# loicland/superpoint_graph

Hardware: NVIDIA H100
Metric: spg_train_step_edges_plus_points_per_sec (higher is better)
Workload: dtype f32

## Files before the change

### superpoint_graph_b200/csrc/tc_gemm2.cu

```cuda
#include <cuda.h>
#include <stdlib.h>

#include <mutex>

#include "common.cuh"
#include "tc_common.cuh"

namespace spg {

constexpr int T2_BM = 128;
constexpr int T2_KC = 32;
constexpr int T2_MAX_STAGES = 4;
constexpr int T2_EPI_WARPS = 8, T2_PROD_WARPS = 8;
constexpr int T2_THREADS = (T2_EPI_WARPS + T2_PROD_WARPS) * 32;
constexpr int T2_A_BYTES = T2_BM * T2_KC * 4;
constexpr int T2_STAGE_BYTES = 2 * T2_A_BYTES;

enum { PRO_AFFINE = 0, PRO_BNBWD = 1 };
enum { EPI_NONE = 0, EPI_STATS = 1, EPI_BNRED = 2 };

struct Tc2Args {
    const float* A;
    int64_t lda;
    const float* A2;
    int64_t lda2;
    const float* bias;
    float* C;
    int64_t ldc;
    int64_t M;
    int N, K;
    const float *a_scale, *a_shift;
    int a_relu;
    const float *a_mean, *a_var, *a_s12;
    float a_eps;
    float* dy_out;
    int64_t lddy;
    int epi;
    float* part;
    float *mean_out, *var_out;
    FoldArgs fold;
    const float* e_y;
    int64_t e_ldy;
    const float *e_scale, *e_shift, *e_mean, *e_var;
    float e_eps;
    int e_relu;
    float* e_s12;
    int nstages;
};

__device__ __forceinline__ void tma_load_2d(uint32_t dst, const CUtensorMap* map, int x, int y, uint32_t bar) {
    asm volatile(
        "cp.async.bulk.tensor.2d.shared::cluster.global.mbarrier::complete_tx::bytes [%0], [%1, {%2, %3}], [%4];"
        ::"r"(dst), "l"(map), "r"(x), "r"(y), "r"(bar)
        : "memory");
}

template <int NS, int PRO>
__global__ void __launch_bounds__(T2_THREADS, 1)
tc_gemm2_kernel(const Tc2Args p, const __grid_constant__ CUtensorMap wmap) {
    extern __shared__ __align__(1024) uint8_t smem_raw[];
    uint8_t* smem = smem_raw;
    if ((smem_u32(smem_raw) & 1023u) != 0u) __trap();
    __shared__ __align__(8) uint64_t bars[2 * T2_MAX_STAGES + 1];

    const int t = threadIdx.x;
    const int warp = t >> 5, lane = t & 31;
    const int nk = p.K / T2_KC;
    const int n0 = blockIdx.y * NS;
    const int64_t tiles = (p.M + T2_BM - 1) / T2_BM;
    const int nst = p.nstages;
    uint8_t* wres = smem + (size_t)nst * T2_STAGE_BYTES;

    const uint32_t bars_u32 = smem_u32(&bars[0]);
    auto bar_full = [&](int s) { return bars_u32 + 8u * (uint32_t)s; };
    auto bar_empty = [&](int s) { return bars_u32 + 8u * (uint32_t)(T2_MAX_STAGES + s); };
    const uint32_t bar_w = bars_u32 + 8u * (2 * T2_MAX_STAGES);

    if (t == 0) {
#pragma unroll
        for (int s = 0; s < T2_MAX_STAGES; ++s) {
            mbar_init(bar_full(s), T2_PROD_WARPS);
            mbar_init(bar_empty(s), T2_EPI_WARPS);
        }
        mbar_init(bar_w, 1);
        asm volatile("fence.mbarrier_init.release.cluster;" ::: "memory");
        asm volatile("prefetch.tensormap [%0];" ::"l"(&wmap) : "memory");
    }
    SPG_PDL_ENTRY();
    if (t == 0) {
        mbar_expect_tx(bar_w, (uint32_t)(nk * 2 * NS * T2_KC * 4));
        const uint32_t wres_u = smem_u32(wres);
        for (int blk = 0; blk < nk * 2; ++blk)
            tma_load_2d(wres_u + (uint32_t)blk * (NS * T2_KC * 4), &wmap, 0, blk * p.N + n0, bar_w);
    }
    constexpr int PF = PRO == PRO_BNBWD ? 2 : 4;
    constexpr int NOPS = PRO == PRO_BNBWD ? 2 : 1;
    float4 q[PF][NOPS][4];
    const int pt = t - T2_EPI_WARPS * 32;
    auto load = [&](int64_t tile, int kc, float4 (&dst)[NOPS][4]) {
        const int64_t m0 = tile * T2_BM;
#pragma unroll
        for (int j = 0; j < 4; ++j) {
            const int i = pt + 256 * j;
            const int row = i >> 3, c16 = i & 7;
            const bool ok = tile < tiles && m0 + row < p.M;
            dst[0][j] = ok ? __ldg(reinterpret_cast<const float4*>(p.A + (m0 + row) * p.lda + kc * T2_KC + c16 * 4))
                           : make_float4(0.f, 0.f, 0.f, 0.f);
            if (PRO == PRO_BNBWD)
                dst[NOPS - 1][j] =
                    ok ? __ldg(reinterpret_cast<const float4*>(p.A2 + (m0 + row) * p.lda2 + kc * T2_KC + c16 * 4))
                       : make_float4(0.f, 0.f, 0.f, 0.f);
        }
    };
    auto advance = [&](int64_t& tl, int& k) {
        if (++k == nk) {
            k = 0;
            tl += gridDim.x;
        }
    };
    int64_t ltile = blockIdx.x;
    int lkc = 0;
    if (pt >= 0) {
#pragma unroll
        for (int d = 0; d < PF - 1; ++d) {
            load(ltile, lkc, q[d]);
            advance(ltile, lkc);
        }
    }
    float* sc_s = reinterpret_cast<float*>(wres + (size_t)nk * 2 * NS * T2_KC * 4);
    float* sh_s = sc_s + p.K;
    float* cy_s = sh_s + p.K;
    float* c0_s = cy_s + p.K;
    float* bias_s = c0_s + p.K;
    float* ev_s = bias_s + NS;
    float* acc_s = ev_s + 4 * NS;
    for (int i = t; i < p.K; i += T2_THREADS) {
        const float sc = p.a_scale ? p.a_scale[i] : 1.f;
        sc_s[i] = sc;
        sh_s[i] = p.a_shift ? p.a_shift[i] : 0.f;
        if (PRO == PRO_BNBWD) {
            const float mu = p.a_mean[i], rstd = 1.f / sqrtf(p.a_var[i] + p.a_eps);
            const float m1 = p.a_s12[i] / (float)p.M, m2 = p.a_s12[p.K + i] / (float)p.M;
            cy_s[i] = -sc * rstd * m2;
            c0_s[i] = sc * (rstd * m2 * mu - m1);
        }
    }
    for (int i = t; i < NS; i += T2_THREADS) {
        bias_s[i] = p.bias ? p.bias[n0 + i] : 0.f;
        if (p.epi == EPI_BNRED) {
            ev_s[i] = p.e_scale ? p.e_scale[n0 + i] : 1.f;
            ev_s[NS + i] = p.e_shift ? p.e_shift[n0 + i] : 0.f;
            ev_s[2 * NS + i] = p.e_mean[n0 + i];
            ev_s[3 * NS + i] = 1.f / sqrtf(p.e_var[n0 + i] + p.e_eps);
        }
    }
    for (int i = t; i < T2_EPI_WARPS * NS * 4; i += T2_THREADS) acc_s[i] = 0.f;
    __syncthreads();

    if (warp >= T2_EPI_WARPS) {
        const bool pro = PRO == PRO_BNBWD || p.a_scale || p.a_shift || p.a_relu;
        int64_t tile = blockIdx.x;
        int kc = 0;
        uint32_t it = 0;
        const int c16 = pt & 7;
        uint32_t soff[4];
#pragma unroll
        for (int j = 0; j < 4; ++j) soff[j] = sw128_off((pt >> 3) + 32 * j, c16);
        const uint32_t smem_u = smem_u32(smem);
        const bool side_store = PRO == PRO_BNBWD && p.dy_out != nullptr && blockIdx.y == 0;
        auto st_shared4 = [](uint32_t addr, uint4 v) {
            asm volatile("st.shared.v4.b32 [%0], {%1, %2, %3, %4};" ::"r"(addr), "r"(v.x), "r"(v.y),
                         "r"(v.z), "r"(v.w)
                         : "memory");
        };
        auto consume = [&](float4 (&cur)[NOPS][4], float4 (&far)[NOPS][4]) {
            const int s = it % nst;
            const uint32_t use = it / nst;
            load(ltile, lkc, far);
            advance(ltile, lkc);
            const int col = kc * T2_KC + c16 * 4;
            const float4 sc = *reinterpret_cast<const float4*>(sc_s + col);
            const float4 sh = *reinterpret_cast<const float4*>(sh_s + col);
            float4 cy = make_float4(0.f, 0.f, 0.f, 0.f), c0 = cy;
            if (PRO == PRO_BNBWD) {
                cy = *reinterpret_cast<const float4*>(cy_s + col);
                c0 = *reinterpret_cast<const float4*>(c0_s + col);
            }
            if (use > 0) mbar_wait(bar_empty(s), (use - 1) & 1);
            const uint32_t stage = smem_u + (uint32_t)s * T2_STAGE_BYTES;
            const int64_t m0 = tile * T2_BM;
#pragma unroll
            for (int j = 0; j < 4; ++j) {
                float4 v = cur[0][j];
                const int64_t row = m0 + (pt >> 3) + 32 * j;
                if (pro && row < p.M) {
                    if (PRO == PRO_BNBWD) {
                        const float4 y = cur[NOPS - 1][j];
                        if (p.a_relu) {
                            if (!(fmaf(y.x, sc.x, sh.x) > 0.f)) v.x = 0.f;
                            if (!(fmaf(y.y, sc.y, sh.y) > 0.f)) v.y = 0.f;
                            if (!(fmaf(y.z, sc.z, sh.z) > 0.f)) v.z = 0.f;
                            if (!(fmaf(y.w, sc.w, sh.w) > 0.f)) v.w = 0.f;
                        }
                        v.x = fmaf(sc.x, v.x, fmaf(cy.x, y.x, c0.x));
                        v.y = fmaf(sc.y, v.y, fmaf(cy.y, y.y, c0.y));
                        v.z = fmaf(sc.z, v.z, fmaf(cy.z, y.z, c0.z));
                        v.w = fmaf(sc.w, v.w, fmaf(cy.w, y.w, c0.w));
                        if (side_store)
                            *reinterpret_cast<float4*>(p.dy_out + row * p.lddy + col) = v;
                    } else {
                        v.x = fmaf(v.x, sc.x, sh.x);
                        v.y = fmaf(v.y, sc.y, sh.y);
                        v.z = fmaf(v.z, sc.z, sh.z);
                        v.w = fmaf(v.w, sc.w, sh.w);
                        if (p.a_relu) {
                            v.x = fmaxf(v.x, 0.f);
                            v.y = fmaxf(v.y, 0.f);
                            v.z = fmaxf(v.z, 0.f);
                            v.w = fmaxf(v.w, 0.f);
                        }
                    }
                }
                uint4 hi, lo;
                hi.x = to_tf32(v.x);
                hi.y = to_tf32(v.y);
                hi.z = to_tf32(v.z);
                hi.w = to_tf32(v.w);
                lo.x = to_tf32(v.x - __uint_as_float(hi.x));
                lo.y = to_tf32(v.y - __uint_as_float(hi.y));
                lo.z = to_tf32(v.z - __uint_as_float(hi.z));
                lo.w = to_tf32(v.w - __uint_as_float(hi.w));
                st_shared4(stage + soff[j], hi);
                st_shared4(stage + T2_A_BYTES + soff[j], lo);
            }
            asm volatile("fence.proxy.async.shared::cta;" ::: "memory");
            __syncwarp();
            if (lane == 0) mbar_arrive(bar_full(s));
            advance(tile, kc);
            ++it;
        };
        while (tile < tiles) {
#pragma unroll
            for (int u = 0; u < PF; ++u) {
                consume(q[u], q[(u + PF - 1) % PF]);
                if (tile >= tiles) break;
            }
        }
    } else {
        const int g = warp >> 2, wl = warp & 3;
        const int r = lane >> 2, cq = 2 * (lane & 3);
        float* acc_w = acc_s + warp * (NS * 4);
        const uint32_t wres_u32 = smem_u32(wres);
        const uint32_t smem_u = smem_u32(smem);
        float acc[NS / 2];
        uint32_t it = 0;
        mbar_wait(bar_w, 0);
        for (int64_t tile = blockIdx.x; tile < tiles; tile += gridDim.x) {
            for (int kc = 0; kc < nk; ++kc, ++it) {
                const int s = it % nst;
                mbar_wait(bar_full(s), (it / nst) & 1);
                const uint32_t a_hi = smem_u + (uint32_t)s * T2_STAGE_BYTES + (uint32_t)g * (64 * 128);
                const uint32_t a_lo = a_hi + T2_A_BYTES;
                const uint32_t b_hi = wres_u32 + (uint32_t)(kc * 2) * (NS * T2_KC * 4);
                const uint32_t b_lo = b_hi + NS * T2_KC * 4;
                wg_reg_fence(acc);
                wg_fence();
#pragma unroll
                for (int ks = 0; ks < T2_KC / 8; ++ks) {
                    const uint32_t ko = ks * 32;
                    const uint64_t dah = wg_desc_k_sw128(a_hi + ko), dal = wg_desc_k_sw128(a_lo + ko);
                    const uint64_t dbh = wg_desc_k_sw128(b_hi + ko), dbl = wg_desc_k_sw128(b_lo + ko);
                    wgmma_tf32<NS>(acc, dah, dbh, (kc | ks) ? 1u : 0u);
                    wgmma_tf32<NS>(acc, dal, dbh, 1u);
                    wgmma_tf32<NS>(acc, dah, dbl, 1u);
                }
                wg_commit();
                wg_wait<0>();
                wg_reg_fence(acc);
                __syncwarp();
                if (lane == 0) mbar_arrive(bar_empty(s));
            }
            const int64_t row0 = tile * T2_BM + g * 64 + wl * 16;
            const int nv = (int)max((int64_t)0, min((int64_t)16, p.M - row0));
            const bool va = r < nv, vb = r + 8 < nv;
            float* ca = p.C + (row0 + r) * p.ldc + n0;
            float* cb = ca + 8 * p.ldc;
#pragma unroll
            for (int j = 0; j < NS / 8; ++j) {
                const int c = 8 * j + cq;
                const float2 oa = make_float2(acc[4 * j] + bias_s[c], acc[4 * j + 1] + bias_s[c + 1]);
                const float2 ob = make_float2(acc[4 * j + 2] + bias_s[c], acc[4 * j + 3] + bias_s[c + 1]);
                if (va) *reinterpret_cast<float2*>(ca + c) = oa;
                if (vb) *reinterpret_cast<float2*>(cb + c) = ob;
                if (p.epi == EPI_BNRED) {
                    const float2 ya = va ? __ldg(reinterpret_cast<const float2*>(p.e_y + (row0 + r) * p.e_ldy + n0 + c))
                                         : make_float2(0.f, 0.f);
                    const float2 yb = vb ? __ldg(reinterpret_cast<const float2*>(p.e_y + (row0 + r + 8) * p.e_ldy + n0 + c))
                                         : make_float2(0.f, 0.f);
                    float b1[2], b2[2];
#pragma unroll
                    for (int e = 0; e < 2; ++e) {
                        const float esc = ev_s[c + e], esh = ev_s[NS + c + e];
                        const float emu = ev_s[2 * NS + c + e], ers = ev_s[3 * NS + c + e];
                        const float y0 = e ? ya.y : ya.x, y1 = e ? yb.y : yb.x;
                        float g0 = va ? (e ? oa.y : oa.x) : 0.f, g1 = vb ? (e ? ob.y : ob.x) : 0.f;
                        if (p.e_relu) {
                            if (!(fmaf(y0, esc, esh) > 0.f)) g0 = 0.f;
                            if (!(fmaf(y1, esc, esh) > 0.f)) g1 = 0.f;
                        }
                        b1[e] = g0 + g1;
                        b2[e] = fmaf(g1, (y1 - emu) * ers, g0 * ((y0 - emu) * ers));
                    }
#pragma unroll
                    for (int e = 0; e < 2; ++e)
#pragma unroll
                        for (int o = 4; o < 32; o <<= 1) {
                            b1[e] += __shfl_xor_sync(0xffffffffu, b1[e], o);
                            b2[e] += __shfl_xor_sync(0xffffffffu, b2[e], o);
                        }
                    if (r == 0) {
#pragma unroll
                        for (int e = 0; e < 2; ++e) {
                            float* o = acc_w + (c + e) * 4;
                            o[0] += b1[e];
                            o[1] += b2[e];
                        }
                    }
                }
                if (p.epi == EPI_STATS && nv > 0) {
#pragma unroll
                    for (int e = 0; e < 2; ++e) {
                        float* o = acc_w + (c + e) * 4;
                        const float n_old = o[0];
                        const float first = __shfl_sync(0xffffffffu, e ? oa.y : oa.x, lane & 3);
                        const float pivot = n_old > 0.f ? o[3] : first;
                        const float d0 = va ? (e ? oa.y : oa.x) - pivot : 0.f;
                        const float d1 = vb ? (e ? ob.y : ob.x) - pivot : 0.f;
                        float s1 = d0 + d1, s2 = fmaf(d1, d1, d0 * d0);
#pragma unroll
                        for (int sh = 4; sh < 32; sh <<= 1) {
                            s1 += __shfl_xor_sync(0xffffffffu, s1, sh);
                            s2 += __shfl_xor_sync(0xffffffffu, s2, sh);
                        }
                        __syncwarp();
                        if (r == 0) {
                            o[0] = n_old + (float)nv;
                            o[1] += s1;
                            o[2] += s2;
                            o[3] = pivot;
                        }
                        __syncwarp();
                    }
                }
            }
        }
    }

    __syncthreads();
    if (p.epi == EPI_NONE) return;

    if (t < NS) {
        if (p.epi == EPI_STATS) {
            double n = 0.0, mean = 0.0, m2 = 0.0;
#pragma unroll
            for (int wq = 0; wq < T2_EPI_WARPS; ++wq) {
                const float* o = acc_s + wq * (NS * 4) + t * 4;
                const double nb = (double)o[0];
                if (nb > 0.0) {
                    const double mb = (double)o[3] + (double)o[1] / nb;
                    const double qb = fmax((double)o[2] - (double)o[1] * (double)o[1] / nb, 0.0);
                    const double tot = n + nb, delta = mb - mean;
                    m2 += qb + delta * delta * n * nb / tot;
                    mean += delta * nb / tot;
                    n = tot;
                }
            }
            float* o = p.part + ((int64_t)blockIdx.x * p.N + n0 + t) * 3;
            o[0] = (float)n;
            o[1] = (float)mean;
            o[2] = (float)m2;
        } else {
            float a1 = 0.f, a2 = 0.f;
#pragma unroll
            for (int wq = 0; wq < T2_EPI_WARPS; ++wq) {
                a1 += acc_s[wq * (NS * 4) + t * 4];
                a2 += acc_s[wq * (NS * 4) + t * 4 + 1];
            }
            float* o = p.part + ((int64_t)blockIdx.x * p.N + n0 + t) * 2;
            o[0] = a1;
            o[1] = a2;
        }
    }
}

__global__ void __launch_bounds__(256) tc_merge_kernel(const Tc2Args p, int P) {
    SPG_PDL_ENTRY();
    const int warp = threadIdx.x >> 5, lane = threadIdx.x & 31;
    const int c = blockIdx.x * 8 + warp;
    if (c >= p.N) return;
    {
        if (p.epi == EPI_STATS) {
            double sn = 0.0, snm = 0.0;
            float pn[5], pm[5], pq[5];
#pragma unroll
            for (int u = 0; u < 5; ++u) {
                const int k = lane + 32 * u;
                pn[u] = pm[u] = pq[u] = 0.f;
                if (k < P) {
                    const float* o = p.part + ((int64_t)k * p.N + c) * 3;
                    pn[u] = __ldcg(o);
                    pm[u] = __ldcg(o + 1);
                    pq[u] = __ldcg(o + 2);
                }
                sn += (double)pn[u];
                snm += (double)pn[u] * (double)pm[u];
            }
#pragma unroll
            for (int o = 16; o > 0; o >>= 1) {
                sn += __shfl_xor_sync(0xffffffffu, sn, o);
                snm += __shfl_xor_sync(0xffffffffu, snm, o);
            }
            const double mu = sn > 0.0 ? snm / sn : 0.0;
            double qq = 0.0;
#pragma unroll
            for (int u = 0; u < 5; ++u) {
                const double d = (double)pm[u] - mu;
                qq += (double)pq[u] + (double)pn[u] * d * d;
            }
#pragma unroll
            for (int o = 16; o > 0; o >>= 1) qq += __shfl_xor_sync(0xffffffffu, qq, o);
            if (lane == 0) {
                const float mu_f = (float)mu;
                const float var_f = sn > 0.0 ? (float)(qq / sn) : 0.f;
                p.mean_out[c] = mu_f;
                p.var_out[c] = var_f;
                if (p.fold.enabled) bn_fold_col(p.fold, c, mu_f, var_f);
            }
        } else {
            double a1 = 0.0, a2 = 0.0;
            for (int k = lane; k < P; k += 32) {
                const float* o = p.part + ((int64_t)k * p.N + c) * 2;
                a1 += (double)__ldcg(o);
                a2 += (double)__ldcg(o + 1);
            }
#pragma unroll
            for (int o = 16; o > 0; o >>= 1) {
                a1 += __shfl_xor_sync(0xffffffffu, a1, o);
                a2 += __shfl_xor_sync(0xffffffffu, a2, o);
            }
            if (lane == 0) {
                p.e_s12[c] = (float)a1;
                p.e_s12[p.N + c] = (float)a2;
            }
        }
    }
}

typedef CUresult (*EncodeTiledFn)(CUtensorMap*, CUtensorMapDataType, cuuint32_t, void*, const cuuint64_t*,
                                  const cuuint64_t*, const cuuint32_t*, const cuuint32_t*,
                                  CUtensorMapInterleave, CUtensorMapSwizzle, CUtensorMapL2promotion,
                                  CUtensorMapFloatOOBfill);

static EncodeTiledFn encode_tiled() {
    static EncodeTiledFn fn = nullptr;
    static std::once_flag once;
    std::call_once(once, [] {
        void* ptr = nullptr;
        cudaDriverEntryPointQueryResult qres;
        if (cudaGetDriverEntryPoint("cuTensorMapEncodeTiled", &ptr, cudaEnableDefault, &qres) == cudaSuccess &&
            qres == cudaDriverEntryPointSuccess)
            fn = reinterpret_cast<EncodeTiledFn>(ptr);
    });
    return fn;
}

static int make_weight_map(CUtensorMap* map, const float* image, int N, int K, int NS) {
    EncodeTiledFn fn = encode_tiled();
    if (!fn) return SPG_E_UNSUPPORTED;
    const cuuint64_t dims[2] = {(cuuint64_t)T2_KC, (cuuint64_t)(K / T2_KC) * 2 * (cuuint64_t)N};
    const cuuint64_t strides[1] = {(cuuint64_t)T2_KC * 4};
    const cuuint32_t box[2] = {(cuuint32_t)T2_KC, (cuuint32_t)NS};
    const cuuint32_t estr[2] = {1, 1};
    const CUresult r = fn(map, CU_TENSOR_MAP_DATA_TYPE_FLOAT32, 2, const_cast<float*>(image), dims, strides, box,
                          estr, CU_TENSOR_MAP_INTERLEAVE_NONE, CU_TENSOR_MAP_SWIZZLE_NONE,
                          CU_TENSOR_MAP_L2_PROMOTION_L2_128B, CU_TENSOR_MAP_FLOAT_OOB_FILL_NONE);
    return r == CUDA_SUCCESS ? SPG_OK : SPG_E_BADARG;
}

static inline int fixed_smem(int NS, int K) {
    return (K / T2_KC) * 2 * NS * T2_KC * 4 + (4 * K + NS + 4 * NS + T2_EPI_WARPS * NS * 4) * 4;
}

static inline int stages_for(int NS, int K) {
    int nst = (232448 - 1024 - fixed_smem(NS, K)) / T2_STAGE_BYTES;
    return nst > T2_MAX_STAGES ? T2_MAX_STAGES : nst;
}

template <int NS, int PRO>
static int launch_tc2(Tc2Args& a, const float* image, cudaStream_t s) {
    const int slices = a.N / NS;
    const int64_t tiles = ceil_div64(a.M, T2_BM);
    int64_t gx = kNumSMs / slices;
    if (gx > tiles) gx = tiles;
    if (gx < 1) gx = 1;
    const int nst = stages_for(NS, a.K);
    if (nst < 2) return SPG_E_UNSUPPORTED;
    a.nstages = nst;
    CUtensorMap map;
    int rc = make_weight_map(&map, image, a.N, a.K, NS);
    if (rc) return rc;
    const int smem = nst * T2_STAGE_BYTES + fixed_smem(NS, a.K);
    cudaError_t e = cudaFuncSetAttribute(tc_gemm2_kernel<NS, PRO>, cudaFuncAttributeMaxDynamicSharedMemorySize, smem);
    if (e != cudaSuccess) return (int)e;
    dim3 grid((unsigned)gx, (unsigned)slices);
    SPG_LAUNCH(K_TC_GEMM, s, (tc_gemm2_kernel<NS, PRO>), grid, T2_THREADS, smem, a, map);
    rc = launch_status();
    if (rc || a.epi == EPI_NONE) return rc;
    SPG_LAUNCH(K_TC_MERGE, s, tc_merge_kernel, (unsigned)ceil_div64(a.N, 8), 256, 0, a, (int)gx);
    return launch_status();
}

static inline int pick_ns(int N, int K) {
    if (N % 128 == 0 && stages_for(128, K) >= 2) return 128;
    if (N % 64 == 0 && stages_for(64, K) >= 2) return 64;
    if (N % 32 == 0 && N <= 64 && stages_for(32, K) >= 2) return 32;
    return 0;
}

}

using namespace spg;

extern "C" {

int spg_tc_gemm_supported(int64_t M, int N, int K) {
    return (M > 0 && N > 0 && N <= 256 && K >= T2_KC && K % T2_KC == 0 && pick_ns(N, K) != 0) ? 1 : 0;
}

int spg_tc_gemm_max_partials(void) { return kNumSMs; }

int spg_tc_gemm_ex(const float* A, int64_t lda, const float* weight_image, const float* bias, float* C,
                   int64_t ldc, int64_t M, int N, int K,
                   const float* a_scale, const float* a_shift, int a_relu,
                   const float* a2, int64_t lda2, const float* a_mean, const float* a_var,
                   const float* a_s12, float a_eps, float* dy_out, int64_t lddy,
                   int epilogue, float* partials_ws,
                   float* mean_out, float* var_out, const float* gamma, const float* beta, float eps,
                   float* scale_out, float* shift_out, float* running_mean, float* running_var,
                   int64_t* num_batches_tracked, float momentum,
                   const float* e_y, int64_t e_ldy, const float* e_scale, const float* e_shift,
                   const float* e_mean, const float* e_var, float e_eps, int e_relu, float* e_s12,
                   spg_stream_t stream) {
    if (M < 0 || !A || !weight_image || !C) return SPG_E_BADARG;
    if (M == 0) return SPG_OK;
    if (!spg_tc_gemm_supported(M, N, K)) return SPG_E_UNSUPPORTED;
    if ((lda & 3) || (ldc & 3) || lda < K || ldc < N) return SPG_E_ALIGN;
    if (((uintptr_t)A | (uintptr_t)C | (uintptr_t)weight_image | (uintptr_t)a2 | (uintptr_t)dy_out |
         (uintptr_t)e_y) & 15)
        return SPG_E_ALIGN;
    if (ceil_div64(M, T2_BM) > 2147483647ll) return SPG_E_UNSUPPORTED;
    Tc2Args a;
    a.A = A; a.lda = lda; a.A2 = a2; a.lda2 = lda2; a.bias = bias; a.C = C; a.ldc = ldc; a.M = M;
    a.N = N; a.K = K; a.a_scale = a_scale; a.a_shift = a_shift; a.a_relu = a_relu;
    a.a_mean = a_mean; a.a_var = a_var; a.a_s12 = a_s12; a.a_eps = a_eps;
    a.dy_out = dy_out; a.lddy = lddy;
    a.epi = epilogue; a.part = partials_ws;
    a.mean_out = mean_out; a.var_out = var_out;
    a.fold = fold_args(gamma, beta, eps, scale_out, shift_out, running_mean, running_var, num_batches_tracked,
                       momentum, M);
    a.e_y = e_y; a.e_ldy = e_ldy; a.e_scale = e_scale; a.e_shift = e_shift; a.e_mean = e_mean;
    a.e_var = e_var; a.e_eps = e_eps; a.e_relu = e_relu; a.e_s12 = e_s12; a.nstages = 0;
    const bool bnbwd = a2 != nullptr;
    if (bnbwd && (!a_scale || !a_shift || !a_mean || !a_var || !a_s12 || (lda2 & 3) || lda2 < K))
        return SPG_E_BADARG;
    if (dy_out && (!bnbwd || (lddy & 3) || lddy < K)) return SPG_E_BADARG;
    if (epilogue == EPI_STATS) {
        if (!partials_ws || !mean_out || !var_out) return SPG_E_BADARG;
        if (a.fold.enabled && !shift_out) return SPG_E_BADARG;
    } else if (epilogue == EPI_BNRED) {
        if (!partials_ws || !e_y || !e_mean || !e_var || !e_s12 || (e_ldy & 3) || e_ldy < N) return SPG_E_BADARG;
    } else if (epilogue != EPI_NONE) {
        return SPG_E_BADARG;
    }
    cudaStream_t s = (cudaStream_t)stream;
    const int ns = pick_ns(N, K);
#define SPG_TC2_CASE(NS_)                                                                  \
    if (ns == NS_) return bnbwd ? launch_tc2<NS_, PRO_BNBWD>(a, weight_image, s)          \
                                : launch_tc2<NS_, PRO_AFFINE>(a, weight_image, s);
    SPG_TC2_CASE(128)
    SPG_TC2_CASE(64)
    SPG_TC2_CASE(32)
#undef SPG_TC2_CASE
    return SPG_E_UNSUPPORTED;
}

int spg_tc_gemm(const float* A, int64_t lda, const float* weight_image, const float* bias, float* C,
                int64_t ldc, int64_t M, int N, int K, const float* a_scale, const float* a_shift,
                int a_relu, spg_stream_t stream) {
    return spg_tc_gemm_ex(A, lda, weight_image, bias, C, ldc, M, N, K, a_scale, a_shift, a_relu, nullptr, 0,
                          nullptr, nullptr, nullptr, 0.f, nullptr, 0, EPI_NONE, nullptr, nullptr, nullptr,
                          nullptr, nullptr, 0.f, nullptr, nullptr, nullptr, nullptr, nullptr, 0.f, nullptr, 0,
                          nullptr, nullptr, nullptr, nullptr, 0.f, 0, nullptr, stream);
}

}
```

Before: 44.96 million.

## Split A ring per warpgroup, ping-pong MMA/epilogue, and reduce-scatter epilogue stats

```diff
diff --git a/superpoint_graph_b200/csrc/tc_gemm2.cu b/superpoint_graph_b200/csrc/tc_gemm2.cu
--- a/superpoint_graph_b200/csrc/tc_gemm2.cu
+++ b/superpoint_graph_b200/csrc/tc_gemm2.cu
@@ -15,6 +15,8 @@
 constexpr int T2_THREADS = (T2_EPI_WARPS + T2_PROD_WARPS) * 32;
 constexpr int T2_A_BYTES = T2_BM * T2_KC * 4;
 constexpr int T2_STAGE_BYTES = 2 * T2_A_BYTES;
+constexpr int T2_HALF_A_BYTES = T2_A_BYTES / 2;
+constexpr int T2_HALF_STAGE_BYTES = 2 * T2_HALF_A_BYTES;
 
 enum { PRO_AFFINE = 0, PRO_BNBWD = 1 };
 enum { EPI_NONE = 0, EPI_STATS = 1, EPI_BNRED = 2 };
@@ -48,6 +50,43 @@
     int nstages;
 };
 
+constexpr int T2_TURN_BAR = 1;
+constexpr int T2_TURN_THREADS = 2 * 128;
+__device__ __forceinline__ void turn_wait(int id) {
+    asm volatile("bar.sync %0, %1;" ::"r"(id), "n"(T2_TURN_THREADS) : "memory");
+}
+__device__ __forceinline__ void turn_pass(int id) {
+    asm volatile("bar.arrive %0, %1;" ::"r"(id), "n"(T2_TURN_THREADS) : "memory");
+}
+
+__device__ __forceinline__ void st_global2(float* ptr, float2 v, bool pred) {
+    asm volatile(
+        "{\n\t.reg .pred p;\n\tsetp.ne.b32 p, %3, 0;\n\t@p st.global.v2.f32 [%0], {%1, %2};\n\t}" ::"l"(ptr),
+        "f"(v.x), "f"(v.y), "r"((int)pred));
+}
+__device__ __forceinline__ void st_global4(float* ptr, float4 v, bool pred) {
+    asm volatile(
+        "{\n\t.reg .pred p;\n\tsetp.ne.b32 p, %5, 0;\n\t@p st.global.v4.f32 [%0], {%1, %2, %3, %4};\n\t}" ::"l"(ptr),
+        "f"(v.x), "f"(v.y), "f"(v.z), "f"(v.w), "r"((int)pred));
+}
+
+__device__ __forceinline__ float reduce_scatter8(const float (&v)[8], int r) {
+    const bool b0 = r & 1, b1 = r & 2, b2 = r & 4;
+    float w[4], x[2];
+#pragma unroll
+    for (int i = 0; i < 4; ++i) {
+        const float keep = b0 ? v[i + 4] : v[i], send = b0 ? v[i] : v[i + 4];
+        w[i] = keep + __shfl_xor_sync(0xffffffffu, send, 4);
+    }
+#pragma unroll
+    for (int i = 0; i < 2; ++i) {
+        const float keep = b1 ? w[i + 2] : w[i], send = b1 ? w[i] : w[i + 2];
+        x[i] = keep + __shfl_xor_sync(0xffffffffu, send, 8);
+    }
+    const float keep = b2 ? x[1] : x[0], send = b2 ? x[0] : x[1];
+    return keep + __shfl_xor_sync(0xffffffffu, send, 16);
+}
+
 __device__ __forceinline__ void tma_load_2d(uint32_t dst, const CUtensorMap* map, int x, int y, uint32_t bar) {
     asm volatile(
         "cp.async.bulk.tensor.2d.shared::cluster.global.mbarrier::complete_tx::bytes [%0], [%1, {%2, %3}], [%4];"
@@ -61,7 +100,7 @@
     extern __shared__ __align__(1024) uint8_t smem_raw[];
     uint8_t* smem = smem_raw;
     if ((smem_u32(smem_raw) & 1023u) != 0u) __trap();
-    __shared__ __align__(8) uint64_t bars[2 * T2_MAX_STAGES + 1];
+    __shared__ __align__(8) uint64_t bars[4 * T2_MAX_STAGES + 1];
 
     const int t = threadIdx.x;
     const int warp = t >> 5, lane = t & 31;
@@ -69,19 +108,22 @@
     const int n0 = blockIdx.y * NS;
     const int64_t tiles = (p.M + T2_BM - 1) / T2_BM;
     const int nst = p.nstages;
+    auto ring = [&](int h) { return smem_u32(smem) + (uint32_t)(h * nst) * T2_HALF_STAGE_BYTES; };
     uint8_t* wres = smem + (size_t)nst * T2_STAGE_BYTES;
 
     const uint32_t bars_u32 = smem_u32(&bars[0]);
-    auto bar_full = [&](int s) { return bars_u32 + 8u * (uint32_t)s; };
-    auto bar_empty = [&](int s) { return bars_u32 + 8u * (uint32_t)(T2_MAX_STAGES + s); };
-    const uint32_t bar_w = bars_u32 + 8u * (2 * T2_MAX_STAGES);
+    auto bar_full = [&](int h, int s) { return bars_u32 + 8u * (uint32_t)(h * T2_MAX_STAGES + s); };
+    auto bar_empty = [&](int h, int s) { return bars_u32 + 8u * (uint32_t)((2 + h) * T2_MAX_STAGES + s); };
+    const uint32_t bar_w = bars_u32 + 8u * (4 * T2_MAX_STAGES);
 
     if (t == 0) {
 #pragma unroll
-        for (int s = 0; s < T2_MAX_STAGES; ++s) {
-            mbar_init(bar_full(s), T2_PROD_WARPS);
-            mbar_init(bar_empty(s), T2_EPI_WARPS);
-        }
+        for (int h = 0; h < 2; ++h)
+#pragma unroll
+            for (int s = 0; s < T2_MAX_STAGES; ++s) {
+                mbar_init(bar_full(h, s), T2_PROD_WARPS / 2);
+                mbar_init(bar_empty(h, s), T2_EPI_WARPS / 2);
+            }
         mbar_init(bar_w, 1);
         asm volatile("fence.mbarrier_init.release.cluster;" ::: "memory");
         asm volatile("prefetch.tensormap [%0];" ::"l"(&wmap) : "memory");
@@ -97,12 +139,12 @@
     constexpr int NOPS = PRO == PRO_BNBWD ? 2 : 1;
     float4 q[PF][NOPS][4];
     const int pt = t - T2_EPI_WARPS * 32;
+    const int ph = pt >> 7, pq = pt & 127;
     auto load = [&](int64_t tile, int kc, float4 (&dst)[NOPS][4]) {
         const int64_t m0 = tile * T2_BM;
 #pragma unroll
         for (int j = 0; j < 4; ++j) {
-            const int i = pt + 256 * j;
-            const int row = i >> 3, c16 = i & 7;
+            const int row = ph * 64 + (pq >> 3) + 16 * j, c16 = pq & 7;
             const bool ok = tile < tiles && m0 + row < p.M;
             dst[0][j] = ok ? __ldg(reinterpret_cast<const float4*>(p.A + (m0 + row) * p.lda + kc * T2_KC + c16 * 4))
                            : make_float4(0.f, 0.f, 0.f, 0.f);
@@ -162,11 +204,11 @@
         int64_t tile = blockIdx.x;
         int kc = 0;
         uint32_t it = 0;
-        const int c16 = pt & 7;
+        const int c16 = pq & 7;
         uint32_t soff[4];
 #pragma unroll
-        for (int j = 0; j < 4; ++j) soff[j] = sw128_off((pt >> 3) + 32 * j, c16);
-        const uint32_t smem_u = smem_u32(smem);
+        for (int j = 0; j < 4; ++j) soff[j] = sw128_off((pq >> 3) + 16 * j, c16);
+        const uint32_t ring_u = ring(ph);
         const bool side_store = PRO == PRO_BNBWD && p.dy_out != nullptr && blockIdx.y == 0;
         auto st_shared4 = [](uint32_t addr, uint4 v) {
             asm volatile("st.shared.v4.b32 [%0], {%1, %2, %3, %4};" ::"r"(addr), "r"(v.x), "r"(v.y),
@@ -186,13 +228,13 @@
                 cy = *reinterpret_cast<const float4*>(cy_s + col);
                 c0 = *reinterpret_cast<const float4*>(c0_s + col);
             }
-            if (use > 0) mbar_wait(bar_empty(s), (use - 1) & 1);
-            const uint32_t stage = smem_u + (uint32_t)s * T2_STAGE_BYTES;
-            const int64_t m0 = tile * T2_BM;
+            if (use > 0) mbar_wait(bar_empty(ph, s), (use - 1) & 1);
+            const uint32_t stage = ring_u + (uint32_t)s * T2_HALF_STAGE_BYTES;
+            const int64_t m0 = tile * T2_BM + ph * 64;
 #pragma unroll
             for (int j = 0; j < 4; ++j) {
                 float4 v = cur[0][j];
-                const int64_t row = m0 + (pt >> 3) + 32 * j;
+                const int64_t row = m0 + (pq >> 3) + 16 * j;
                 if (pro && row < p.M) {
                     if (PRO == PRO_BNBWD) {
                         const float4 y = cur[NOPS - 1][j];
@@ -206,8 +248,7 @@
                         v.y = fmaf(sc.y, v.y, fmaf(cy.y, y.y, c0.y));
                         v.z = fmaf(sc.z, v.z, fmaf(cy.z, y.z, c0.z));
                         v.w = fmaf(sc.w, v.w, fmaf(cy.w, y.w, c0.w));
-                        if (side_store)
-                            *reinterpret_cast<float4*>(p.dy_out + row * p.lddy + col) = v;
+                        st_global4(p.dy_out + row * p.lddy + col, v, side_store);
                     } else {
                         v.x = fmaf(v.x, sc.x, sh.x);
                         v.y = fmaf(v.y, sc.y, sh.y);
@@ -231,11 +272,11 @@
                 lo.z = to_tf32(v.z - __uint_as_float(hi.z));
                 lo.w = to_tf32(v.w - __uint_as_float(hi.w));
                 st_shared4(stage + soff[j], hi);
-                st_shared4(stage + T2_A_BYTES + soff[j], lo);
+                st_shared4(stage + T2_HALF_A_BYTES + soff[j], lo);
             }
             asm volatile("fence.proxy.async.shared::cta;" ::: "memory");
             __syncwarp();
-            if (lane == 0) mbar_arrive(bar_full(s));
+            if (lane == 0) mbar_arrive(bar_full(ph, s));
             advance(tile, kc);
             ++it;
         };
@@ -251,16 +292,18 @@
         const int r = lane >> 2, cq = 2 * (lane & 3);
         float* acc_w = acc_s + warp * (NS * 4);
         const uint32_t wres_u32 = smem_u32(wres);
-        const uint32_t smem_u = smem_u32(smem);
+        const uint32_t ring_u = ring(g);
         float acc[NS / 2];
+        float n_w = 0.f;
         uint32_t it = 0;
         mbar_wait(bar_w, 0);
         for (int64_t tile = blockIdx.x; tile < tiles; tile += gridDim.x) {
+            if (g == 1 || tile != blockIdx.x) turn_wait(T2_TURN_BAR + g);
             for (int kc = 0; kc < nk; ++kc, ++it) {
                 const int s = it % nst;
-                mbar_wait(bar_full(s), (it / nst) & 1);
-                const uint32_t a_hi = smem_u + (uint32_t)s * T2_STAGE_BYTES + (uint32_t)g * (64 * 128);
-                const uint32_t a_lo = a_hi + T2_A_BYTES;
+                mbar_wait(bar_full(g, s), (it / nst) & 1);
+                const uint32_t a_hi = ring_u + (uint32_t)s * T2_HALF_STAGE_BYTES;
+                const uint32_t a_lo = a_hi + T2_HALF_A_BYTES;
                 const uint32_t b_hi = wres_u32 + (uint32_t)(kc * 2) * (NS * T2_KC * 4);
                 const uint32_t b_lo = b_hi + NS * T2_KC * 4;
                 wg_reg_fence(acc);
@@ -278,80 +321,88 @@
                 wg_wait<0>();
                 wg_reg_fence(acc);
                 __syncwarp();
-                if (lane == 0) mbar_arrive(bar_empty(s));
-            }
+                if (lane == 0) mbar_arrive(bar_empty(g, s));
+            }
+            if (g == 0 || tile + gridDim.x < tiles) turn_pass(T2_TURN_BAR + (g ^ 1));
             const int64_t row0 = tile * T2_BM + g * 64 + wl * 16;
             const int nv = (int)max((int64_t)0, min((int64_t)16, p.M - row0));
             const bool va = r < nv, vb = r + 8 < nv;
             float* ca = p.C + (row0 + r) * p.ldc + n0;
             float* cb = ca + 8 * p.ldc;
-#pragma unroll
-            for (int j = 0; j < NS / 8; ++j) {
-                const int c = 8 * j + cq;
-                const float2 oa = make_float2(acc[4 * j] + bias_s[c], acc[4 * j + 1] + bias_s[c + 1]);
-                const float2 ob = make_float2(acc[4 * j + 2] + bias_s[c], acc[4 * j + 3] + bias_s[c + 1]);
-                if (va) *reinterpret_cast<float2*>(ca + c) = oa;
-                if (vb) *reinterpret_cast<float2*>(cb + c) = ob;
+            const bool have_pivot = n_w > 0.f;
+            if (p.epi == EPI_STATS) __syncwarp();
+            const bool reduce = p.epi == EPI_BNRED || (p.epi == EPI_STATS && nv > 0);
+            const int vr = 4 * (r & 1) + 2 * ((r >> 1) & 1) + (r >> 2);
+            constexpr int YB = NS == 128 ? 2 : 4;
+#pragma unroll
+            for (int j1 = 0; j1 < NS / 8; j1 += YB) {
+                float2 ya[YB], yb[YB];
                 if (p.epi == EPI_BNRED) {
-                    const float2 ya = va ? __ldg(reinterpret_cast<const float2*>(p.e_y + (row0 + r) * p.e_ldy + n0 + c))
-                                         : make_float2(0.f, 0.f);
-                    const float2 yb = vb ? __ldg(reinterpret_cast<const float2*>(p.e_y + (row0 + r + 8) * p.e_ldy + n0 + c))
-                                         : make_float2(0.f, 0.f);
-                    float b1[2], b2[2];
-#pragma unroll
-                    for (int e = 0; e < 2; ++e) {
-                        const float esc = ev_s[c + e], esh = ev_s[NS + c + e];
-                        const float emu = ev_s[2 * NS + c + e], ers = ev_s[3 * NS + c + e];
-                        const float y0 = e ? ya.y : ya.x, y1 = e ? yb.y : yb.x;
-                        float g0 = va ? (e ? oa.y : oa.x) : 0.f, g1 = vb ? (e ? ob.y : ob.x) : 0.f;
-                        if (p.e_relu) {
-                            if (!(fmaf(y0, esc, esh) > 0.f)) g0 = 0.f;
-                            if (!(fmaf(y1, esc, esh) > 0.f)) g1 = 0.f;
+#pragma unroll
+                    for (int u = 0; u < YB; ++u) {
+                        const int64_t col = n0 + 8 * (j1 + u) + cq;
+                        ya[u] = va ? __ldg(reinterpret_cast<const float2*>(p.e_y + (row0 + r) * p.e_ldy + col))
+                                   : make_float2(0.f, 0.f);
+                        yb[u] = vb ? __ldg(reinterpret_cast<const float2*>(p.e_y + (row0 + r + 8) * p.e_ldy + col))
+                                   : make_float2(0.f, 0.f);
+                    }
+                }
+#pragma unroll
+                for (int j0 = j1; j0 < j1 + YB; j0 += 2) {
+                    float v[8];
+                    float piv[4];
+#pragma unroll
+                    for (int u = 0; u < 2; ++u) {
+                        const int j = j0 + u;
+                        const int c = 8 * j + cq;
+                        const float2 oa = make_float2(acc[4 * j] + bias_s[c], acc[4 * j + 1] + bias_s[c + 1]);
+                        const float2 ob = make_float2(acc[4 * j + 2] + bias_s[c], acc[4 * j + 3] + bias_s[c + 1]);
+                        st_global2(ca + c, oa, va);
+                        st_global2(cb + c, ob, vb);
+#pragma unroll
+                        for (int e = 0; e < 2; ++e) {
+                            const int k = 2 * u + e;
+                            if (p.epi == EPI_BNRED) {
+                                const float esc = ev_s[c + e], esh = ev_s[NS + c + e];
+                                const float emu = ev_s[2 * NS + c + e], ers = ev_s[3 * NS + c + e];
+                                const float2 y0p = ya[j - j1], y1p = yb[j - j1];
+                                const float y0 = e ? y0p.y : y0p.x, y1 = e ? y1p.y : y1p.x;
+                                float g0 = va ? (e ? oa.y : oa.x) : 0.f, g1 = vb ? (e ? ob.y : ob.x) : 0.f;
+                                if (p.e_relu) {
+                                    if (!(fmaf(y0, esc, esh) > 0.f)) g0 = 0.f;
+                                    if (!(fmaf(y1, esc, esh) > 0.f)) g1 = 0.f;
+                                }
+                                v[2 * k] = g0 + g1;
+                                v[2 * k + 1] = fmaf(g1, (y1 - emu) * ers, g0 * ((y0 - emu) * ers));
+                            } else if (p.epi == EPI_STATS && nv > 0) {
+                                const float x0 = e ? oa.y : oa.x, x1 = e ? ob.y : ob.x;
+                                const float first = __shfl_sync(0xffffffffu, x0, lane & 3);
+                                piv[k] = have_pivot ? acc_w[(c + e) * 4 + 3] : first;
+                                const float d0 = va ? x0 - piv[k] : 0.f;
+                                const float d1 = vb ? x1 - piv[k] : 0.f;
+                                v[2 * k] = d0 + d1;
+                                v[2 * k + 1] = fmaf(d1, d1, d0 * d0);
+                            }
                         }
-                        b1[e] = g0 + g1;
-                        b2[e] = fmaf(g1, (y1 - emu) * ers, g0 * ((y0 - emu) * ers));
                     }
-#pragma unroll
-                    for (int e = 0; e < 2; ++e)
-#pragma unroll
-                        for (int o = 4; o < 32; o <<= 1) {
-                            b1[e] += __shfl_xor_sync(0xffffffffu, b1[e], o);
-                            b2[e] += __shfl_xor_sync(0xffffffffu, b2[e], o);
-                        }
-                    if (r == 0) {
-#pragma unroll
-                        for (int e = 0; e < 2; ++e) {
-                            float* o = acc_w + (c + e) * 4;
-                            o[0] += b1[e];
-                            o[1] += b2[e];
+                    if (reduce) {
+                        const float sum = reduce_scatter8(v, r);
+                        const int k = vr >> 1;
+                        acc_w[(8 * (j0 + (k >> 1)) + cq + (k & 1)) * 4 + (p.epi == EPI_STATS) + (vr & 1)] += sum;
+                        if (p.epi == EPI_STATS && r == 0 && !have_pivot) {
+#pragma unroll
+                            for (int q = 0; q < 4; ++q) acc_w[(8 * (j0 + (q >> 1)) + cq + (q & 1)) * 4 + 3] = piv[q];
                         }
                     }
                 }
-                if (p.epi == EPI_STATS && nv > 0) {
-#pragma unroll
-                    for (int e = 0; e < 2; ++e) {
-                        float* o = acc_w + (c + e) * 4;
-                        const float n_old = o[0];
-                        const float first = __shfl_sync(0xffffffffu, e ? oa.y : oa.x, lane & 3);
-                        const float pivot = n_old > 0.f ? o[3] : first;
-                        const float d0 = va ? (e ? oa.y : oa.x) - pivot : 0.f;
-                        const float d1 = vb ? (e ? ob.y : ob.x) - pivot : 0.f;
-                        float s1 = d0 + d1, s2 = fmaf(d1, d1, d0 * d0);
-#pragma unroll
-                        for (int sh = 4; sh < 32; sh <<= 1) {
-                            s1 += __shfl_xor_sync(0xffffffffu, s1, sh);
-                            s2 += __shfl_xor_sync(0xffffffffu, s2, sh);
-                        }
-                        __syncwarp();
-                        if (r == 0) {
-                            o[0] = n_old + (float)nv;
-                            o[1] += s1;
-                            o[2] += s2;
-                            o[3] = pivot;
-                        }
-                        __syncwarp();
-                    }
-                }
+            }
+            if (p.epi == EPI_STATS && nv > 0) n_w += (float)nv;
+        }
+        if (p.epi == EPI_STATS && r == 0) {
+#pragma unroll
+            for (int j = 0; j < NS / 8; ++j) {
+                acc_w[(8 * j + cq) * 4] = n_w;
+                acc_w[(8 * j + cq + 1) * 4] = n_w;
             }
         }
     }
```

After: 47.55 million, median of 6. 5.8% higher.
